# mhozza/covest

Hardware: AMD Instinct MI355X
Metric: grid-point log-likelihood evals/s, repeat model, 10k-bin hist (higher is better)
Workload: dtype f64

## Files before the change

### covest_amd/csrc/ll_factored.hip

```cpp
#include <hip/hip_runtime.h>

#include <algorithm>
#include <mutex>
#include <type_traits>

#include "direct_point.h"
#include "fastmath.h"
#include "kernels.h"
#include "point_fetch.h"
#include "streams.h"
#include "wave.h"

namespace covest {

namespace {

typedef double d4 __attribute__((ext_vector_type(4)));

constexpr double kShareScale = 0x1p128;


template <int N, int MU>
__device__ __forceinline__ void contract_step(int i, const double *cur, const int (&a_off)[MU], const int (&cut)[MU],
                                              const double (&r4)[MU], double (&wrun)[MU], d4 (&acc)[MU])
{
    double a[N];
#pragma unroll
    for (int k = 0; k < N; ++k)
        a[k] = cur[a_off[k] + 4 * i];
#pragma unroll
    for (int k = 0; k < N; ++k) {
        const double w = (i < cut[k]) ? wrun[k] : 0.0;
        wrun[k] *= r4[k];
        acc[k] = __builtin_amdgcn_mfma_f64_16x16x4f64(a[k], w, acc[k], 0, 0, 0);
    }
}

[[maybe_unused]] constexpr int kLdWide = 290;
template <int NT, int HU, bool TAIL, bool PLAIN, int LDC = 0>
__global__ __launch_bounds__(NT) void ll_factored_kernel(const DevModel m, const int32_t n_tiles, const int32_t n_items,
                                                         const double *__restrict__ tile_dbl,
                                                         const int32_t *__restrict__ tile_int,
                                                         const FactoredPlan plan,
                                                         double *__restrict__ out_ll, const SubList sub_list)
{
    const TileView tv = tile_view_from(n_tiles, n_items, tile_dbl, tile_int);
#ifdef COVEST_DIAG
    const long long dgx_0 = (long long)clock64();
    long long dgx_1 = 0, dgx_2 = 0, dgx_3 = 0, dgx_4 = 0;
#endif
    constexpr int NW = NT / kWave;
    constexpr int MU = 2 * HU;
    static_assert(MU == 6, "contract loops are written for 6 slots");
    constexpr bool SPO = PLAIN && TAIL;
    constexpr bool NEED_SCAL = !PLAIN;
    constexpr int LOG_DEG = PLAIN ? 3 : 5;
    const int LD = LDC ? LDC : plan.ld;
    constexpr int NE = FactoredLds::entries_of(NT);
    const FactoredLds lay{NT, plan.n_buf, LD, SPO};
    extern __shared__ double Gs[];
    __shared__ __attribute__((aligned(16))) double log_tab[kLogTableDoubles];
    __shared__ unsigned sub_rec[NE * 2];
    __shared__ __attribute__((aligned(16))) double2 rowc[2][kTileBins];
    __shared__ __attribute__((aligned(16))) double rows[NEED_SCAL ? 2 : 1][NEED_SCAL ? kTileBins : 2];
    __shared__ __attribute__((aligned(16))) double rho_tab[PLAIN ? NW * MU * 4 : 4];
    __shared__ double lconst_s;
    static_assert(MU == kMaxUnits, "the LDS layout counts kMaxUnits slots a wave");
    static_assert(sizeof(log_tab) + sizeof(sub_rec) + sizeof(rowc) + sizeof(rows) + sizeof(rho_tab) + sizeof(lconst_s) + 6 * 15 <=
                      kFactoredStaticLds, "the planners' LDS budget (tiles.h) must hold the kernel's static LDS");

    const int tid = threadIdx.x;
    const int lane = tid & (kWave - 1);
    const int wave = __builtin_amdgcn_readfirstlane(tid / kWave);
    const double p_clamp = plan.p_clamp;
    const double zero_frac = kZeroSteps * (kGridStep / p_clamp);
    const int list_mode = PLAIN ? 0 : plan.list_mode;

    const int n_seg = list_mode ? plan.n_seg : 1;
    const int unit = list_mode ? (int)blockIdx.x / n_seg : (int)blockIdx.x;
    const int seg = list_mode ? (int)blockIdx.x - unit * n_seg : 0;
    const int seg_items = (n_items + n_seg - 1) / n_seg;
    const int t_begin = seg * seg_items, t_end = min(n_items, t_begin + seg_items);
    const int64_t ce = (PLAIN || list_mode == 0) ? plan.ce_end - 1 - unit : plan.ce_begin + unit;
    const bool list = list_mode == 1 || list_mode == 2;
    const int64_t ic = list ? ce : ce / plan.n_e;
    const int64_t ie = list ? ce : ce - ic * plan.n_e;
    double par[kMaxParams] = {plan.c_axis[ic], plan.e_axis[ie], 0, 0, 0};
    constexpr int kLogPerThread = (kLogTableDoubles + NT - 1) / NT;
    double log_v[kLogPerThread];
#pragma unroll
    for (int u = 0; u < kLogPerThread; ++u)
        log_v[u] = kLogTable[min(tid + u * NT, kLogTableDoubles - 1)];
    const double rho_v = PLAIN ? plan.unit_rho[(int64_t)blockIdx.y * NW * MU * 4 + min(tid, NW * MU * 4 - 1)] : 0.0;
    double lc_first = 0.0;
    if (wave == NW - 1 && t_begin + lane < t_end)
        lc_first = tv.item_lconst[t_begin + lane];
#pragma unroll
    for (int u = 0; u < kLogPerThread; ++u)
        if (tid + u * NT < kLogTableDoubles)
            log_tab[tid + u * NT] = log_v[u];
    if (PLAIN && tid < NW * MU * 4)
        rho_tab[tid] = rho_v;
#pragma unroll
    for (int u = 0; u < (NE + NT - 1) / NT; ++u)
        if (tid + u * NT < NE) {
            sub_rec[2 * (tid + u * NT)] = 0xFFFFFFFFu;
            sub_rec[2 * (tid + u * NT) + 1] = 0;
        }
    clamp_point<2>(m, par);
    const bool finite = isfinite(par[0]) && isfinite(par[1]);
    const int n_pass = PLAIN ? 1 : plan.n_pass;
    if (tid < 8 * n_pass)
        Gs[lay.rates() + tid] = error_class_rate_mul(m, par[0], par[1], tid, m.n_err);
    if (wave == NW - 1) {
        double lc = 0.0 + lc_first;
        for (int t = t_begin + lane + kWave; t < t_end; t += kWave)
            lc += tv.item_lconst[t];
        lc = wave_sum(lc);
        if (lane == 0)
            lconst_s = PLAIN ? lc - kLogRawBias<kScaleBits> * tv.suf_h[0] : lc;
    }
    __syncthreads();
#ifdef COVEST_DIAG
    dgx_1 = (long long)clock64();
#endif

    const int my_pass = n_pass == 1 ? 0 : tid / plan.pass_stride;
    const int o_local = n_pass == 1 ? tid : tid - my_pass * plan.pass_stride;
    const bool wave_builds = wave * kWave < plan.n_columns;
    const int o_base = PLAIN ? 0 : list_mode == 2 ? plan.item_obase[ce] : plan.o_base;
    const int o_mine = o_base + o_local + 1;
    double lam[8];
#pragma unroll
    for (int s = 0; s < 8; ++s)
        lam[s] = Gs[lay.rates() + 8 * my_pass + s];
    double n_total = -1.0;
    if (n_pass > 1) {
        n_total = 0.0;
        for (int s = 0; s < 8 * n_pass; ++s)
            n_total += m.comb[s] * (1.0 - exp_neg_rn((double)o_mine * Gs[lay.rates() + s]));
    }
    __syncthreads();
    StreamSet<8> st;
    if (wave_builds) {
        st.template init<false>(m, lam, o_mine, finite && my_pass < n_pass && o_local < plan.max_o, log_tab,
                                log_tab, 8 * my_pass, n_total);
    } else {
        st.gone = 0u;
#pragma unroll
        for (int s = 0; s < 8; ++s) {
            st.v[s] = 0.0;
            st.x[s] = 0.0;
            st.an.set(s, 0.0, -INFINITY);
        }
    }
#ifdef COVEST_DIAG
    dgx_2 = (long long)clock64();
#endif
    const bool lane_in_row = tid < LD - 2;
    if (tid < FactoredLds::kSlack)
        Gs[lay.slack() + tid] = 0.0;
    if (tid < lay.rows()) {
        Gs[lay.pad(tid)] = 0.0;
        Gs[lay.pad(tid) + 1] = 0.0;
    }

    const int col = lane & 15;
    const int kq = lane >> 4;
    int len[MU], cont[MU], uhalf[MU], qslot[MU], cut[MU], a_off0[MU], nsh[MU];
    double r4[MU], llacc[MU];
    uint64_t dead[MU];
    unsigned off_slots = 0;
    bool newly_dead = false;
    CompSum spacc[(TAIL && !SPO) ? MU : 1];
    CompSum so = {0.0, 0.0};
    auto wave_block = [&](int w) -> int {
        if (list)
            return w >= NW - 2 ? 1 + 2 * (int)ce + (w - (NW - 2)) : 0;
        return (int)blockIdx.y * NW + w;
    };
    const int slot_base = wave_block(wave) * MU;
    int u_qt[MU], u_s0[MU], u_len[MU], u_cont[MU], u_half[MU], u_nsh[MU], u_o0[MU], u_T[MU];
#pragma unroll
    for (int k = 0; k < MU; ++k) {
        const int at = slot_base + k;
        u_qt[k] = plan.unit_tile[at];
        u_s0[k] = plan.unit_s0[at];
        u_len[k] = plan.unit_len[at];
        u_cont[k] = plan.unit_cont[at];
        u_half[k] = plan.unit_half[at];
        u_nsh[k] = PLAIN ? plan.unit_nsh[at] : 0;
        u_o0[k] = plan.unit_o0[at];
    }
#pragma unroll
    for (int k = 0; k < MU; ++k) {
        const int qt = __builtin_amdgcn_readfirstlane(u_qt[k]);
        const bool on = qt >= 0;
        const int slot = (on ? qt : 0) * 16 + col;
        qslot[k] = on ? slot : -1;
        u_T[k] = plan.q_T[slot];
        r4[k] = plan.q_r4[slot];
    }
#pragma unroll
    for (int k = 0; k < MU; ++k) {
        const bool on = qslot[k] >= 0;
        const int first_step = __builtin_amdgcn_readfirstlane(u_s0[k]);
        len[k] = __builtin_amdgcn_readfirstlane(u_len[k]);
        cont[k] = __builtin_amdgcn_readfirstlane(u_cont[k]);
        uhalf[k] = __builtin_amdgcn_readfirstlane(u_half[k]);
        nsh[k] = PLAIN ? __builtin_amdgcn_readfirstlane(u_nsh[k]) : 0;
        a_off0[k] = (16 * uhalf[k] + col) * LD + kq + 4 * first_step;
        const int t_lane = on ? u_T[k] : 0;
        const int o0 = __builtin_amdgcn_readfirstlane(u_o0[k]);
        cut[k] = ((t_lane - (o0 + kq) + 3) >> 2) - nsh[k];
        llacc[k] = 0.0;
        dead[k] = 0;
        spacc[(TAIL && !SPO) ? k : 0].hi = 0.0;
        spacc[(TAIL && !SPO) ? k : 0].lo = 0.0;
    }

    unsigned m_first = 0, m_cont = 0, m_sh = 0;
#pragma unroll
    for (int k = 0; k < MU; ++k) {
        m_first |= (qslot[k] >= 0 && !cont[k]) ? 1u << k : 0u;
        m_cont |= cont[k] ? 1u << k : 0u;
        m_sh |= nsh[k] > 0 ? 1u << k : 0u;
    }
    double wfirst[MU], wrun[MU];
    auto load_weights = [&]() {
#pragma unroll
        for (int k = 0; k < MU; ++k) {
            const double2 pw = reinterpret_cast<const double2 *>(plan.piece_w)[(int64_t)(slot_base + k) * kWave + lane];
            wfirst[k] = pw.x;
            wrun[k] = pw.y;
        }
    };
    load_weights();

    long long dg_a = 0, dg_b = 0, dg_b0 = 0, dg_c = 0, dg_w = 0, dg_t0 = 0, dg_zero = 0, dg_enter = 0, dg_first = 0;
#ifdef COVEST_DIAG
    const bool diag = plan.diag != nullptr;
#else
    constexpr bool diag = false;
#endif
    auto walk_tile = [&](auto n_tag, double *colp, double renorm, double k0) __attribute__((always_inline)) -> double {
        constexpr int N = decltype(n_tag)::value;
        if (!lane_in_row)
            return 0.0;
        double xx[8];
#pragma unroll
        for (int s = 0; s < 8; ++s) {
            double xs = st.x[s];
            if (s < N) {
                asm volatile("" : "+v"(xs));
                xx[s] = xs * xs;
            } else {
                xx[s] = 0.0;
            }
        }
        double *row = colp;
        double tsum = 0.0;
        if (SPO) {
            double kk = k0;
#pragma unroll
            for (int b = 0; b < kTileBins; b += 2) {
                double g1, g2;
                st.template step2n<N>(xx, g1, g2);
                row[0] = g1;
                row[LD] = g2;
                row += 2 * LD;
                tsum = fma(tsum, kk, g1);
                kk += 1.0;
                tsum = fma(tsum, kk, g2);
                kk += 1.0;
            }
            tsum *= renorm;
        } else {
#pragma unroll
            for (int b = 0; b < kTileBins; b += 2) {
                double g1, g2;
                st.template step2n<N>(xx, g1, g2);
                row[0] = g1;
                row[LD] = g2;
                row += 2 * LD;
            }
        }
        st.template leave_tile_n<N>(renorm);
        return tsum;
    };
    auto build_tile = [&](int t, bool seg_start, double *dst) __attribute__((always_inline)) -> double {
        if (COVEST_SKIP_PHASE(plan, 1))
            return 0.0;
        const TileRec rc = tv.rec[t];
        const double k0 = rc.k0;
        const int nb = rc.nb;
        const int n_live = st.enter_tile(k0 - 1.0, k0 + (double)(nb - 1), rc.lgam_prev, rc.lgam_last,
                                         rc.run_start != 0 || seg_start);
        if (diag) {
            const long long now__ = (long long)clock64();
            dg_enter += now__ - dg_t0;
            dg_t0 = now__;
        }
        double *colp = dst + (lane_in_row ? tid : 0);
        const double *scal = tv.scal + (int64_t)t * kTileBins;
        if (nb == kTileBins && !(SPO && rc.has_filler != 0)) {
            if (n_live > 4)
                return walk_tile(std::integral_constant<int, 8>{}, colp, rc.renorm, k0);
            if (n_live > 2)
                return walk_tile(std::integral_constant<int, 4>{}, colp, rc.renorm, k0);
            if (n_live == 2)
                return walk_tile(std::integral_constant<int, 2>{}, colp, rc.renorm, k0);
            if (n_live == 1)
                return walk_tile(std::integral_constant<int, 1>{}, colp, rc.renorm, k0);
            if (lane_in_row) {
                if (diag)
                    dg_zero += 1;
#pragma unroll
                for (int b = 0; b < kTileBins; ++b)
                    colp[b * LD] = 0.0;
            }
            return 0.0;
        }
        double tsum = 0.0;
        for (int b = 0; b < kTileBins; ++b) {
            const double g = b < nb ? st.step() : 0.0;
            if (SPO && b < nb)
                tsum = fma(g, scal[b], tsum);
            if (lane_in_row)
                colp[b * LD] = g;
        }
        st.leave_tile(rc.renorm);
        return tsum * 0x1p476;
    };
    auto sum_tile = [&](auto n_tag, const double *scal_ptr, double scal_or_k0, double renorm) __attribute__((always_inline)) -> double {
        constexpr int N = decltype(n_tag)::value;
        double xx[8];
#pragma unroll
        for (int s = 0; s < 8; ++s) {
            double xs = st.x[s];
            if (s < N) {
                asm volatile("" : "+v"(xs));
                xx[s] = xs * xs;
            } else {
                xx[s] = 0.0;
            }
        }
        double gsum = 0.0;
        if (SPO) {
            double kk = scal_or_k0;
#pragma unroll
            for (int b = 0; b < kTileBins; b += 2) {
                double g1, g2;
                st.template step2n<N>(xx, g1, g2);
                gsum = fma(gsum, kk, g1);
                kk += 1.0;
                gsum = fma(gsum, kk, g2);
                kk += 1.0;
            }
            st.template leave_tile_n<N>(renorm);
            return gsum * renorm;
        }
        const double *scal = SPO ? nullptr : scal_ptr;
#pragma unroll
        for (int half = 0; half < 2; ++half) {
            double sc[16];
#pragma unroll
            for (int b = 0; b < 16; ++b)
                sc[b] = scal[16 * half + b];
            asm volatile("" ::: "memory");
#pragma unroll
            for (int b = 0; b < 16; b += 2) {
                double g1, g2;
                st.template step2n<N>(xx, g1, g2);
                gsum = fma(g1, sc[b], gsum);
                gsum = fma(g2, sc[b + 1], gsum);
            }
        }
        st.template leave_tile_n<N>(renorm);
        return gsum * (1.0 / kBasicScale);
    };
    auto build_tile_sum = [&](int t, bool seg_start) __attribute__((always_inline)) -> double {
        const TileRec rc = tv.rec[t];
        const double k0 = rc.k0;
        const int nb = rc.nb;
        const int n_live = SPO ? st.enter_sum_tile(k0 - 1.0, k0 + (double)(nb - 1), rc.lgam_prev, rc.lgam_last,
                                                   rc.run_start != 0 || seg_start)
                               : st.enter_tile(k0 - 1.0, k0 + (double)(nb - 1), rc.lgam_prev, rc.lgam_last,
                                               rc.run_start != 0 || seg_start);
        const double *scal = tv.scal + (int64_t)t * kTileBins;
        if (nb == kTileBins && !(SPO && rc.has_filler != 0)) {
            if (n_live > 2)
                return sum_tile(std::integral_constant<int, 8>{}, scal, k0, rc.renorm);
            if (n_live == 2)
                return sum_tile(std::integral_constant<int, 2>{}, scal, k0, rc.renorm);
            if (n_live == 1)
                return sum_tile(std::integral_constant<int, 1>{}, scal, k0, rc.renorm);
            return 0.0;
        }
        double gsum = 0.0;
        for (int b = 0; b < nb; ++b)
            gsum = fma(st.step(), scal[b], gsum);
        st.leave_tile(rc.renorm);
        return SPO ? gsum * 0x1p476 : gsum * (1.0 / kBasicScale);
    };
    bool resync = false;
    auto build_item = [&](int it, bool seg_start, double *dst) __attribute__((always_inline)) {
        const int first = TAIL ? __builtin_amdgcn_readfirstlane(tv.item_first[it]) : it;
        if (TAIL && tv.item_sum[it] != 0) {
            if (COVEST_SKIP_PHASE(plan, 1))
                return;
            const int n = __builtin_amdgcn_readfirstlane(tv.item_ntiles[it]);
            if (SPO) {
                if (!seg_start) {
                    const int tl = first + n - 1;
                    const TileRec ra = tv.rec[first], rb = tv.rec[tl];
                    const double ka = ra.k0 - 1.0, kb = rb.k0 + (double)(rb.nb - 1);
                    const double lga = ra.lgam_prev, lgb = rb.lgam_last;
                    bool matters = false;
#pragma unroll
                    for (int s = 0; s < 8; ++s) {
                        if ((st.gone >> s) & 1u)
                            continue;
                        const double lx = st.an.lx(s), c = st.an.c(s);
                        const double top = fmax(fma(ka, lx, c - lga), fma(kb, lx, c - lgb));
                        matters = matters || !(top < StreamSet<8>::kSumWindowLn) || (st.x[s] >= ka - 1.0 && st.x[s] <= kb + 1.0);
                    }
                    if (!__any(matters)) {
#pragma unroll
                        for (int s = 0; s < 8; ++s)
                            st.v[s] = 0.0;
                        resync = true;
                        return;
                    }
                }
                for (int r = 0; r < n; ++r) {
                    if (st.gone == 0xFFu && !(seg_start && r == 0))
                        break;
                    so.add(build_tile_sum(first + r, (seg_start && r == 0) || resync));
                    resync = false;
                }
                return;
            }
            double *colp = dst + (lane_in_row ? tid : 0);
            for (int r = 0; r < n; ++r) {
                const double gsum = build_tile_sum(first + r, seg_start && r == 0);
                if (lane_in_row)
                    colp[r * LD] = gsum;
            }
            for (int r = n; r < kTileBins; ++r)
                if (lane_in_row)
// ... 473 lines not shown
    }
    ll = wave_sum(ll);
    double tail_term = 0.0;
    if (m.tail != 0.0) {
        double s = wave_comp_sum(sp);
        if (!(s < 1.0))
            s = 1.0;
        if (s < 1.0)
            tail_term = m.tail * log(1.0 - s);
    }
    if (__ballot(dead))
        ll = isnan(ll) ? ll : -INFINITY;
    double v = ll + tail_term;
    if (__ballot(poisoned) || !(isfinite(par[0]) && isfinite(par[1])))
        v = NAN;
    return v;
}

__global__ __launch_bounds__(kWave) void ll_finish_partials(const DevModel m, const int32_t n_tiles, const int32_t n_items,
                                                           const double *__restrict__ tile_dbl,
                                                           const int32_t *__restrict__ tile_int,
                                                           const double *__restrict__ partial,
                                                           const int32_t *__restrict__ first_item,
                                                           const double *__restrict__ point_par,
                                                           const int32_t *__restrict__ point_T, double *__restrict__ out_ll)
{
    const TileView tv = tile_view_from(n_tiles, n_items, tile_dbl, tile_int);
    const int p = blockIdx.x;
    const int c0 = first_item[p], c1 = first_item[p + 1];
    const int64_t n_rows = (int64_t)n_items * kTileBins;
    double par[kMaxParams];
#pragma unroll
    for (int d = 0; d < kMaxParams; ++d)
        par[d] = point_par[(int64_t)p * kMaxParams + d];
    clamp_point<5>(m, par);
    const double v = finish_point(m, tv, par, point_T[p], [&](int64_t row) {
        double pj = 0.0;
        for (int c = c0; c < c1; ++c)
            pj += partial[(int64_t)c * n_rows + row];
        return pj;
    });
    if (threadIdx.x == 0)
        out_ll[p] = v;
}

__global__ __launch_bounds__(kWave) void ll_finish_dense(const DevModel m, const int32_t n_tiles, const int32_t n_items,
                                                        const double *__restrict__ tile_dbl,
                                                        const int32_t *__restrict__ tile_int, const PointSource src,
                                                        const double *__restrict__ partial, const int64_t ce_first,
                                                        const int64_t n_cols, const int32_t *__restrict__ q_orig,
                                                        const int64_t n_q, const int64_t flat_end,
                                                        double *__restrict__ out_ll)
{
    const TileView tv = tile_view_from(n_tiles, n_items, tile_dbl, tile_int);
    const int64_t ce_local = blockIdx.x / n_cols, slot = blockIdx.x - ce_local * n_cols;
    const int32_t qo = q_orig[slot];
    if (qo < 0)
        return;
    const int64_t flat = (ce_first + ce_local) * n_q + qo;
    if (flat < src.flat_begin || flat >= flat_end)
        return;
    double par[kMaxParams];
    int T;
    fetch_point<5>(src, flat - src.flat_begin, par, T);
    clamp_point<5>(m, par);
    const int64_t n_rows = (int64_t)n_items * kTileBins;
    const double *mine = partial + (ce_local * n_cols + slot) * n_rows;
    const double v = finish_point(m, tv, par, T, [&](int64_t row) { return mine[row]; });
    if (threadIdx.x == 0)
        out_ll[flat - src.flat_begin] = v;
}

#endif

}

inline int64_t factored_rows_per_launch(const FactoredPlan &plan) { return std::max<int64_t>(1, ((int64_t)1 << 22) / plan.n_qblocks); }

template <int NT, bool TAIL, bool PLAIN, int LDC = 0>
hipError_t launch_ll_factored_variant(const DevModel &m, const TileView &tv, const FactoredPlan &plan,
                                      double *out_ll, const SubList &sub_list, hipStream_t stream)
{
    constexpr int HU = kHalfUnits;
    const FactoredLds lay{NT, plan.n_buf, plan.ld, PLAIN && TAIL};
    if (!lay.fits())
        return hipErrorInvalidValue;
    const size_t lds = (size_t)lay.total() * sizeof(double);
    static size_t configured[64] = {0};
    static std::mutex configured_lock;
    std::lock_guard<std::mutex> guard(configured_lock);
    int dev = 0;
    if (hipGetDevice(&dev) != hipSuccess || dev < 0 || dev >= 64)
        dev = 0;
    if (lds > configured[dev]) {
        hipError_t e = hipFuncSetAttribute(reinterpret_cast<const void *>(&ll_factored_kernel<NT, HU, TAIL, PLAIN, LDC>),
                                           hipFuncAttributeMaxDynamicSharedMemorySize, (int)lds);
        if (e != hipSuccess)
            return e;
        configured[dev] = lds;
    }
    const int64_t per_launch = factored_rows_per_launch(plan);
    for (int64_t first = plan.ce_begin; first < plan.ce_end; first += per_launch) {
        FactoredPlan part = plan;
        part.ce_begin = first;
        part.ce_end = std::min(plan.ce_end, first + per_launch);
        const dim3 grid((unsigned)((part.ce_end - part.ce_begin) * (plan.list_mode ? plan.n_seg : 1)),
                        (unsigned)plan.n_qblocks);
        hipLaunchKernelGGL((ll_factored_kernel<NT, HU, TAIL, PLAIN, LDC>), grid, dim3(NT), lds, stream, m, tv.n_tiles, tv.n_items,
                           tv.dbl_base, tv.int_base, part, out_ll, sub_list);
    }
    return hipGetLastError();
}

#ifdef COVEST_FACTORED_VARIANT
#if COVEST_FACTORED_VARIANT >= 8
template hipError_t launch_ll_factored_variant<512, (COVEST_FACTORED_VARIANT & 1) != 0, true, kLdWide>(
    const DevModel &, const TileView &, const FactoredPlan &, double *, const SubList &, hipStream_t);
#else
template hipError_t launch_ll_factored_variant<(COVEST_FACTORED_VARIANT & 4) ? 512 : 256, (COVEST_FACTORED_VARIANT & 2) != 0,
                                               (COVEST_FACTORED_VARIANT & 1) != 0>(const DevModel &, const TileView &,
                                                                                   const FactoredPlan &, double *,
                                                                                   const SubList &, hipStream_t);
#endif
#else
extern template hipError_t launch_ll_factored_variant<256, false, false>(const DevModel &, const TileView &, const FactoredPlan &, double *, const SubList &, hipStream_t);
extern template hipError_t launch_ll_factored_variant<256, false, true>(const DevModel &, const TileView &, const FactoredPlan &, double *, const SubList &, hipStream_t);
extern template hipError_t launch_ll_factored_variant<256, true, false>(const DevModel &, const TileView &, const FactoredPlan &, double *, const SubList &, hipStream_t);
extern template hipError_t launch_ll_factored_variant<256, true, true>(const DevModel &, const TileView &, const FactoredPlan &, double *, const SubList &, hipStream_t);
extern template hipError_t launch_ll_factored_variant<512, false, false>(const DevModel &, const TileView &, const FactoredPlan &, double *, const SubList &, hipStream_t);
extern template hipError_t launch_ll_factored_variant<512, false, true>(const DevModel &, const TileView &, const FactoredPlan &, double *, const SubList &, hipStream_t);
extern template hipError_t launch_ll_factored_variant<512, true, false>(const DevModel &, const TileView &, const FactoredPlan &, double *, const SubList &, hipStream_t);
extern template hipError_t launch_ll_factored_variant<512, true, true>(const DevModel &, const TileView &, const FactoredPlan &, double *, const SubList &, hipStream_t);
extern template hipError_t launch_ll_factored_variant<512, false, true, kLdWide>(const DevModel &, const TileView &, const FactoredPlan &, double *, const SubList &, hipStream_t);
extern template hipError_t launch_ll_factored_variant<512, true, true, kLdWide>(const DevModel &, const TileView &, const FactoredPlan &, double *, const SubList &, hipStream_t);
const char *const kFactoredVariantNames[kFactoredVariants] = {
    "ll_factored<256>", "ll_factored<256,plain>", "ll_factored<256,tail>", "ll_factored<256,tail,plain>",
    "ll_factored<512>", "ll_factored<512,plain>", "ll_factored<512,tail>", "ll_factored<512,tail,plain>",
    "ll_factored<512,plain,ld290>", "ll_factored<512,tail,plain,ld290>"};
const char *const kFactoredFinishNames[2] = {"ll_finish_dense", "ll_finish_partials"};
static_assert(kLdWide == 290, "kFactoredVariantNames spell the row stride of kLdWide");

namespace {

constexpr bool lds_overlap(int a0, int a1, int b0, int b1) { return a0 < b1 && b0 < a1; }
constexpr bool factored_lds_sound()
{
    for (int nt = 256; nt <= 512; nt += 256)
        for (int n_buf = 1; n_buf <= 2; ++n_buf)
            for (int k = 1; k <= 17; ++k)
                for (int spo = 0; spo <= 1; ++spo)
                    for (int t_end = 1; t_end <= 2; ++t_end) {
                        const FactoredLds l{nt, n_buf, kTileBins * k + 2, spo != 0};
                        const int ne = l.entries(), total = l.total();
                        if (l.buf(n_buf - 1) + kTileBins * l.ld > l.slack() || l.slack() + FactoredLds::kSlack > total ||
                            l.rates() + FactoredLds::kRates > total || l.pad(l.rows() - 1) + 2 > l.slack())
                            return false;
                        if (l.part_ll() + ne > total || l.part_hi(t_end) + ne > total || l.part_lo(t_end) + ne > total ||
                            lds_overlap(l.part_ll(), l.part_ll() + ne, l.part_hi(t_end), l.part_lo(t_end) + ne))
                            return false;
                        if (spo) {
                            const int s0 = l.spo_parts(t_end), s1 = s0 + 2 * ne, live = l.buf(t_end);
                            if (s1 > total || lds_overlap(s0, s1, l.slack(), l.slack() + FactoredLds::kSlack) ||
                                lds_overlap(s0, s1, live, live + (n_buf == 2 ? kTileBins : 2) * l.ld))
                                return false;
                            const int other = l.buf(t_end + 1);
                            if (n_buf == 2 && s0 < l.slack() && (s0 < other || s1 > other + kTileBins * l.ld))
                                return false;
                        }
                        if (factored_n_buf(l.ld) == n_buf && !l.fits())
                            return false;
                    }
    return true;
}
static_assert(factored_lds_sound(), "K-factored's LDS layout (tiles.h FactoredLds)");
static_assert(FactoredLds{512, 2, kLdWide, false}.total() == 2 * kTileBins * kLdWide + FactoredLds::kSlack, "C3's LDS");

template <int NT>
hipError_t launch_nt(const DevModel &m, const TileView &tv, const FactoredPlan &plan, double *out_ll,
                     const SubList &sub_list, hipStream_t stream)
{
    const bool plain = plan.list_mode == 0 && plan.n_pass == 1;
    {
        const bool tail = m.tail != 0.0;
        const int v = NT == 512 && plain && plan.ld == kLdWide ? 8 + (tail ? 1 : 0)
                                                                : (NT == 512 ? 4 : 0) + (tail ? 2 : 0) + (plain ? 1 : 0);
        const int64_t rows = plan.ce_end - plan.ce_begin, per_launch = factored_rows_per_launch(plan);
        record_launch(kFactoredVariantNames[v], (rows + per_launch - 1) / per_launch);
    }
    if (NT == 512 && plain && plan.ld == kLdWide)
        return m.tail != 0.0 ? launch_ll_factored_variant<512, true, true, kLdWide>(m, tv, plan, out_ll, sub_list, stream)
                             : launch_ll_factored_variant<512, false, true, kLdWide>(m, tv, plan, out_ll, sub_list, stream);
    if (m.tail != 0.0)
        return plain ? launch_ll_factored_variant<NT, true, true>(m, tv, plan, out_ll, sub_list, stream)
                     : launch_ll_factored_variant<NT, true, false>(m, tv, plan, out_ll, sub_list, stream);
    return plain ? launch_ll_factored_variant<NT, false, true>(m, tv, plan, out_ll, sub_list, stream)
                 : launch_ll_factored_variant<NT, false, false>(m, tv, plan, out_ll, sub_list, stream);
}

}

hipError_t launch_ll_finish_partials(const DevModel &m, const TileView &tv, const double *partial,
                                     const int32_t *first_item, const double *point_par, const int32_t *point_T,
                                     int64_t n_points, double *out_ll, hipStream_t stream)
{
    if (n_points <= 0)
        return hipSuccess;
    record_launch(kFactoredFinishNames[1]);
    hipLaunchKernelGGL(ll_finish_partials, dim3((unsigned)n_points), dim3(kWave), 0, stream, m, tv.n_tiles, tv.n_items, tv.dbl_base,
                       tv.int_base, partial, first_item, point_par, point_T, out_ll);
    return hipGetLastError();
}

hipError_t launch_ll_finish_dense(const DevModel &m, const TileView &tv, const PointSource &src, const double *partial,
                                  int64_t ce_first, int64_t n_ce, int64_t n_cols, const int32_t *q_orig, int64_t n_q,
                                  int64_t flat_end, double *out_ll, hipStream_t stream)
{
    const int64_t per_launch = std::max<int64_t>(1, ((int64_t)1 << 24) / n_cols);
    for (int64_t first = 0; first < n_ce; first += per_launch) {
        const int64_t cnt = std::min(per_launch, n_ce - first);
        record_launch(kFactoredFinishNames[0]);
        hipLaunchKernelGGL(ll_finish_dense, dim3((unsigned)(cnt * n_cols)), dim3(kWave), 0, stream, m, tv.n_tiles, tv.n_items,
                           tv.dbl_base, tv.int_base, src, partial + first * n_cols * (int64_t)tv.n_items * kTileBins,
                           ce_first + first, n_cols, q_orig, n_q, flat_end, out_ll);
    }
    return hipGetLastError();
}

hipError_t launch_ll_factored(const DevModel &m, const TileView &tv, const FactoredPlan &plan,
                              double *out_ll, const SubList &sub_list, hipStream_t stream)
{
    if (plan.ce_end <= plan.ce_begin)
        return hipSuccess;
    if (m.kind != 1 || plan.n_columns > plan.n_threads || 8 * plan.n_pass < m.n_err)
        return hipErrorInvalidValue;
    if (plan.n_threads == 256 && plan.half_units == 3)
        return launch_nt<256>(m, tv, plan, out_ll, sub_list, stream);
    if (plan.n_threads == 512 && plan.half_units == 3)
        return launch_nt<512>(m, tv, plan, out_ll, sub_list, stream);
    return hipErrorInvalidValue;
}
#endif

}
```

### covest_amd/csrc/streams.h

```cpp
#pragma once
#include <hip/hip_runtime.h>

#include "device_model.h"
#include "fastmath.h"
#include "point_fetch.h"
#include "tiles.h"

namespace covest {

template <int S>
struct RegAnchors {
    double lx_[S], c_[S];
    __device__ __forceinline__ void set(int s, double lx, double c) { lx_[s] = lx; c_[s] = c; }
    __device__ __forceinline__ double lx(int s) const { return lx_[s]; }
    __device__ __forceinline__ double c(int s) const { return c_[s]; }
};

template <int S>
struct LdsAnchors {
    double *mine;
    int stride;
    __device__ __forceinline__ void set(int s, double lx, double c)
    {
        mine[(2 * s) * stride] = lx;
        mine[(2 * s + 1) * stride] = c;
    }
    __device__ __forceinline__ double lx(int s) const { return mine[(2 * s) * stride]; }
    __device__ __forceinline__ double c(int s) const { return mine[(2 * s + 1) * stride]; }
};

template <int S, class Anchors = RegAnchors<S>>
struct StreamSet {
    double v[S];
    double x[S];
    Anchors an;
    unsigned gone;

    template <bool CANCEL = true>
    __device__ __forceinline__ void init(const DevModel &m, const double *lam, int o, bool live, const double *log_tab,
                                         const double *norm_tab = nullptr, int s0 = 0, double total = -1.0)
    {
        double n_os[S];
        double tot = 0.0;
        gone = 0u;
#pragma unroll
        for (int s = 0; s < S; ++s) {
            x[s] = (double)o * lam[s];
            n_os[s] = m.comb[s0 + s] * (1.0 - exp_neg_rn(x[s]));
            tot += n_os[s];
        }
        if (total >= 0.0)
            tot = total;
        if (tot == 0.0)
            tot = 1.0;
        const double ln_tot = CANCEL ? fast_log(tot, log_tab) : 0.0;
#pragma unroll
        for (int s = 0; s < S; ++s) {
            v[s] = 0.0;
            if (live && x[s] > 0.0 && n_os[s] > 0.0) {
                const double lx = fast_log(x[s], log_tab);
                double c;
                if (CANCEL ? x[s] < 0.015625 : true) {
                    const double a = n_os[s] / tot;
                    c = a > 0.0 ? fast_log(a, log_tab) - log_trunc_norm(x[s], lx, norm_tab) : -INFINITY;
                } else if (x[s] <= 200.0) {
                    c = (m.ln_comb[s0 + s] - ln_tot) - x[s];
                } else {
                    c = (m.ln_comb[s0 + s] - ln_tot) - log_trunc_norm(x[s], lx, norm_tab);
                }
                if (c == -INFINITY)
                    x[s] = 0.0;
                an.set(s, c == -INFINITY ? 0.0 : lx, c);
            } else {
                x[s] = 0.0;
                an.set(s, 0.0, -INFINITY);
            }
        }
    }

    __device__ __forceinline__ int enter_tile(double km1, double klast, double lgam_prev,
                                              double lgam_last, bool run_start)
    {
        return enter_tile_n<S>(km1, klast, lgam_prev, lgam_last, run_start);
    }

    static constexpr double kSumWindowLn = -60.0;
    __device__ __forceinline__ int enter_sum_tile(double km1, double klast, double lgam_prev, double lgam_last, bool run_start)
    {
        return enter_tile_n<S, true>(km1, klast, lgam_prev, lgam_last, run_start);
    }

    template <int N, bool SUM_ONLY = false>
    __device__ __forceinline__ int enter_tile_n(double km1, double klast, double lgam_prev,
                                                double lgam_last, bool run_start)
    {
        uint64_t m_window[N], m_need[N], m_real[SUM_ONLY ? N : 1];
        double a0s[N];
        uint64_t any_need = 0;
#pragma unroll
        for (int s = 0; s < N; ++s) {
            m_window[s] = m_need[s] = 0;
            a0s[s] = 0.0;
            if ((gone >> s) & 1u)
                continue;
            const double lx = an.lx(s), c = an.c(s);
            const double a0 = fma(km1, lx, c - lgam_prev);
            const double a1 = fma(klast, lx, c - lgam_last);
            const double top = fmax(a0, a1);
            m_window[s] = __ballot(top > (SUM_ONLY ? kSumWindowLn : kWindowLn));
            if (SUM_ONLY) {
                m_real[s] = __ballot(top > kWindowLn);
                v[s] = (!(top > kSumWindowLn) && km1 >= x[s]) ? 0.0 : v[s];
            }
            m_need[s] = run_start ? m_window[s] : (__ballot(v[s] == 0.0) & m_window[s]);
            if (run_start)
                v[s] = 0.0;
            a0s[s] = a0;
            any_need |= m_need[s];
        }
        if (any_need != 0) {
            const uint64_t me = 1ull << (threadIdx.x & 63);
#pragma unroll
            for (int s = 0; s < N; ++s) {
                if (m_need[s] == 0)
                    continue;
                const double anchored = exp_scaled(a0s[s], kScaleBits);
                v[s] = (m_need[s] & me) ? anchored : v[s];
            }
        }
        int n_live = 0;
#pragma unroll
        for (int s = 0; s < N; ++s) {
            if ((gone >> s) & 1u)
                continue;
            const uint64_t m_on = __ballot(v[s] != 0.0);
            const uint64_t m_stay = (SUM_ONLY ? m_real[s] : m_window[s]) | __ballot(!(km1 >= x[s]));
            if (m_on != 0)
                n_live = s + 1;
            else if (m_stay == 0)
                gone |= 1u << s;
        }
        return n_live;
    }

    __device__ __forceinline__ void retire_at_run_start(double km1, double klast, double lgam_prev, double lgam_last)
    {
#pragma unroll
        for (int s = 0; s < S; ++s) {
            if ((gone >> s) & 1u)
                continue;
            const double lx = an.lx(s), c = an.c(s);
            const double a0 = fma(km1, lx, c - lgam_prev);
            const double a1 = fma(klast, lx, c - lgam_last);
            const bool in_window = fmax(a0, a1) > kWindowLn;
            if (!__any(in_window || !(km1 >= x[s]))) {
                gone |= 1u << s;
                v[s] = 0.0;
            }
        }
    }

    __device__ __forceinline__ double step()
    {
        v[0] *= x[0];
        double g = v[0];
#pragma unroll
        for (int s = 1; s < S; ++s) {
            v[s] *= x[s];
            g += v[s];
        }
        return g;
    }

    __device__ __forceinline__ void step2(const double (&xx)[S], double &g1, double &g2)
    {
        g1 = v[0] * x[0];
#pragma unroll
        for (int s = 1; s < S; ++s)
            g1 = fma(v[s], x[s], g1);
        v[0] *= xx[0];
        g2 = v[0];
#pragma unroll
        for (int s = 1; s < S; ++s) {
            v[s] *= xx[s];
            g2 += v[s];
        }
    }

    template <int N>
    __device__ __forceinline__ void step2n(const double (&xx)[S], double &g1, double &g2)
    {
        static_assert(N >= 1 && N <= S, "live streams");
        g1 = v[0] * x[0];
#pragma unroll
        for (int s = 1; s < N; ++s)
            g1 = fma(v[s], x[s], g1);
        v[0] *= xx[0];
        g2 = v[0];
#pragma unroll
        for (int s = 1; s < N; ++s) {
            v[s] *= xx[s];
            g2 += v[s];
        }
    }

    template <int N>
    __device__ __forceinline__ double step_n()
    {
        v[0] *= x[0];
        double g = v[0];
#pragma unroll
        for (int s = 1; s < N; ++s) {
            v[s] *= x[s];
            g += v[s];
        }
        return g;
    }

    __device__ __forceinline__ bool only_first_left() const { return (gone | 1u) == (~0u >> (32 - S)); }

    template <int N>
    __device__ __forceinline__ void leave_tile_n(double renorm)
    {
#pragma unroll
        for (int s = 0; s < N; ++s)
            v[s] *= renorm;
    }

    __device__ __forceinline__ void squares(double (&xx)[S]) const
    {
#pragma unroll
        for (int s = 0; s < S; ++s)
            xx[s] = x[s] * x[s];
    }

    __device__ __forceinline__ void leave_tile(double renorm)
    {
#pragma unroll
        for (int s = 0; s < S; ++s)
            v[s] *= renorm;
    }
};

}
```

### covest_amd/csrc/tiles.h

```cpp
#pragma once
#include <hip/hip_runtime_api.h>
#include <stdint.h>

namespace covest {

constexpr int kTileBins = 32;
constexpr int kScaleBits = 540;
constexpr double kScaleLn = 540.0 * 0.693147180559945309417232121458;
constexpr double kWindowLn = -760.0;
constexpr int kBasicShift = 64;
constexpr double kBasicScale = 0x1p64;

struct alignas(64) TileRec {
    double k0, lgam_prev, lgam_last, renorm;
    int32_t nb, run_start, all_zero, has_filler;
    double pad[2];
};
static_assert(sizeof(TileRec) == 64, "one cache line");

struct TileView {
    int32_t n_tiles;
    int32_t n_items;
    const double *dbl_base;
    const int32_t *int_base;
    const double *first_key;
    const int32_t *n_bins;
    const int32_t *run_start;
    const int32_t *all_zero;
    const int32_t *has_filler;
    const double *lgam_prev;
    const double *lgam_last;
    const double *renorm;
    const double *scal;
    const double *cnt;
    const double *item_cnt;
    const double *item_scal;
    const double *item_iscal;
    const double *item_lconst;
    const double *suf_h;
    const double *suf_jh;
    const double *suf_lgh;
    const double *suf_first;
    const double *suf_first_lg;
    const double *last_key;
    const int32_t *item_first;
    const int32_t *item_ntiles;
    const int32_t *item_sum;
    const int32_t *row_bin;
    const TileRec *rec;
};

inline __host__ __device__ int64_t tile_arrays_dbl(int32_t nt, int32_t ni)
{
    const int64_t n = 4 * (int64_t)nt + 2 * (int64_t)nt * kTileBins + 3 * (int64_t)ni * kTileBins + ni + 5 * ((int64_t)nt + 1) + 2;
    return (n + 7) / 8 * 8;
}
inline __host__ __device__ int64_t tile_dbl_count(int32_t nt, int32_t ni) { return tile_arrays_dbl(nt, ni) + 8 * (int64_t)nt; }
inline __host__ __device__ int64_t tile_int_count(int32_t nt, int32_t ni) { return 4 * (int64_t)nt + 3 * (int64_t)ni + (int64_t)nt * kTileBins; }

inline __host__ __device__ TileView tile_view_from(int32_t nt, int32_t ni, const double *dbl, const int32_t *ints)
{
    TileView tv;
    tv.n_tiles = nt;
    tv.n_items = ni;
    tv.dbl_base = dbl;
    tv.int_base = ints;
    tv.first_key = dbl;
    tv.lgam_prev = dbl + nt;
    tv.lgam_last = dbl + 2 * (int64_t)nt;
    tv.renorm = dbl + 3 * (int64_t)nt;
    tv.scal = dbl + 4 * (int64_t)nt;
    tv.cnt = tv.scal + (int64_t)nt * kTileBins;
    tv.item_cnt = tv.cnt + (int64_t)nt * kTileBins;
    tv.item_scal = tv.item_cnt + (int64_t)ni * kTileBins;
    tv.item_iscal = tv.item_scal + (int64_t)ni * kTileBins;
    tv.item_lconst = tv.item_iscal + (int64_t)ni * kTileBins;
    tv.suf_h = tv.item_lconst + ni;
    tv.suf_jh = tv.suf_h + (nt + 1);
    tv.suf_lgh = tv.suf_jh + (nt + 1);
    tv.suf_first = tv.suf_lgh + (nt + 1);
    tv.suf_first_lg = tv.suf_first + (nt + 1);
    tv.last_key = tv.suf_first_lg + (nt + 1);
    tv.n_bins = ints;
    tv.run_start = ints + nt;
    tv.all_zero = ints + 2 * (int64_t)nt;
    tv.has_filler = ints + 3 * (int64_t)nt;
    tv.item_first = ints + 4 * (int64_t)nt;
    tv.item_ntiles = tv.item_first + ni;
    tv.item_sum = tv.item_ntiles + ni;
    tv.row_bin = tv.item_sum + ni;
    tv.rec = reinterpret_cast<const TileRec *>(dbl + tile_arrays_dbl(nt, ni));
    return tv;
}

constexpr int kMaxUnits = 6;
constexpr int kHalfUnits = 3;
constexpr int kBuildCost = 18;
constexpr int kBuildCostLowKeys = 24;
constexpr int kLowKeyTile = 384;
#ifndef COVEST_LIST_SEGMENTS
#define COVEST_LIST_SEGMENTS 16
#endif
constexpr int kListSegments = COVEST_LIST_SEGMENTS;
constexpr int kMinPieceSteps = 6;
constexpr int kSharedStepsPerMfma = 4;
constexpr int kMinSharedSteps = 3;
constexpr int kLastBuilderExtra = 4;
constexpr int kUnitOverhead = 2;

struct FactoredPlan {
    const double *c_axis, *e_axis;
    int64_t n_e;
    int64_t ce_begin, ce_end;
    int64_t n_q;
    int32_t n_qtiles;
    int32_t max_o;
    int32_t n_pass;
    int32_t pass_stride;
    int32_t n_columns;
    int32_t o_base;
    int32_t n_threads;
    int32_t half_units;
    int32_t n_qblocks;
    int32_t ld;
    int32_t n_buf;
    const int32_t *unit_tile;
    const int32_t *unit_half;
    const int32_t *unit_s0;
    const int32_t *unit_o0;
    const int32_t *unit_len;
    const int32_t *unit_cont;
    const int32_t *unit_nsh;
    const int32_t *unit_pair;
    const double *unit_rho;
    const double *piece_w;
    const int32_t *qtile_nsteps;
    const int32_t *qtile_nfull;
    const int32_t *q_T;
    const int32_t *q_orig;
    const double *q_first8;
    const double *q_r4;
    int64_t flat_begin, flat_end;
    int32_t list_mode;
    double p_clamp;
    int32_t n_seg;
    const int32_t *item_obase;
    double *partial;
    int64_t ce_first;
    int64_t n_cols_partial;
    long long *diag;
    int32_t skip_phases;
};

constexpr int kLdsBytes = 160 * 1024;
constexpr int kFactoredStaticLds = 13440;

constexpr __host__ __device__ int factored_ld(int columns) { return (columns + kTileBins - 1) / kTileBins * kTileBins + 2; }

struct FactoredLds {
    int nt, n_buf, ld;
    bool spo;
    static constexpr int kSlack = 64;
    static constexpr int kRates = 32;
    __host__ __device__ static constexpr int entries_of(int nt) { return nt / 64 * kMaxUnits * 16; }
    __host__ __device__ constexpr int entries() const { return entries_of(nt); }
    __host__ __device__ constexpr int rows() const { return n_buf * kTileBins; }
    __host__ __device__ constexpr int buf(int b) const { return n_buf == 2 ? (b & 1) * kTileBins * ld : 0; }
    __host__ __device__ constexpr int pad(int row) const { return row * ld + ld - 2; }
    __host__ __device__ constexpr int slack() const { return n_buf * kTileBins * ld; }
    __host__ __device__ constexpr int rates() const { return 0; }
    __host__ __device__ constexpr bool spo_inside() const
    {
        return kTileBins * ld >= (n_buf == 2 ? 0 : 2 * ld) + 3 * entries();
    }
    __host__ __device__ constexpr int spo_parts(int t_end) const
    {
        return !spo_inside() ? slack() + kSlack : n_buf == 2 ? buf(t_end + 1) + entries() : 2 * ld + entries();
    }
    __host__ __device__ constexpr int part_ll() const { return 0; }
    __host__ __device__ constexpr int part_hi(int t_end) const { return spo ? spo_parts(t_end) : entries(); }
    __host__ __device__ constexpr int part_lo(int t_end) const { return part_hi(t_end) + entries(); }
    __host__ __device__ constexpr int total() const
    {
        const int a = slack() + kSlack, b = 3 * entries(), c = spo && !spo_inside() ? slack() + kSlack + 2 * entries() : 0;
        return a > b ? (a > c ? a : c) : (b > c ? b : c);
    }
    __host__ __device__ constexpr bool fits() const { return total() * (int)sizeof(double) + kFactoredStaticLds <= kLdsBytes; }
};

constexpr __host__ __device__ int factored_n_buf(int ld) { return FactoredLds{512, 2, ld, true}.fits() ? 2 : 1; }

#ifdef COVEST_DIAG
#define COVEST_SKIP_PHASE(plan, bits) (((plan).skip_phases & (bits)) != 0)
#else
#define COVEST_SKIP_PHASE(plan, bits) false
#endif

}
```

Measured before the change: 398.1 million.

## Add per-tile relative window table to skip negligible streams in plain kernel

Adds a pre-pass in the plain factored kernel where each building wave scans tiles and records, per tile, the largest log-term margin over the window from reference lanes, using an LDS table updated with atomicMax. When entering a tile, streams whose top term falls below that reference minus a fixed margin (about 100 bits) are excluded from the window, so fewer streams are live and fewer walk_tile steps run. The cost is an extra per-block pass over tiles with atomics and a barrier, plus 128 more LDS doubles. There is a risk of dropping terms if the margin argument does not hold.

```diff
diff --git a/covest_amd/csrc/ll_factored.hip b/covest_amd/csrc/ll_factored.hip
--- a/covest_amd/csrc/ll_factored.hip
+++ b/covest_amd/csrc/ll_factored.hip
@@ -37,6 +37,7 @@
 }
 
 [[maybe_unused]] constexpr int kLdWide = 290;
+[[maybe_unused]] constexpr double kWindowMargin = 100.0 * 0.693147180559945309417232121458 + 2.07944154167983592825169636437;
 template <int NT, int HU, bool TAIL, bool PLAIN, int LDC = 0>
 __global__ __launch_bounds__(NT) void ll_factored_kernel(const DevModel m, const int32_t n_tiles, const int32_t n_items,
                                                          const double *__restrict__ tile_dbl,
@@ -101,6 +102,8 @@
             log_tab[tid + u * NT] = log_v[u];
     if (PLAIN && tid < NW * MU * 4)
         rho_tab[tid] = rho_v;
+    if (PLAIN && tid < FactoredLds::kWinTiles)
+        Gs[lay.win() + tid] = 0.0;
 #pragma unroll
     for (int u = 0; u < (NE + NT - 1) / NT; ++u)
         if (tid + u * NT < NE) {
@@ -153,6 +156,34 @@
             st.x[s] = 0.0;
             st.an.set(s, 0.0, -INFINITY);
         }
+    }
+    if (PLAIN) {
+        if (wave_builds) {
+            unsigned long long *wtab = reinterpret_cast<unsigned long long *>(Gs + lay.win());
+            const double lx0 = st.an.lx(0), c0 = st.an.c(0), x0 = st.x[0], lam0 = lam[0];
+            const bool ref_lane = o_mine >= 3 && x0 > 0.0;
+            const bool lowest = o_mine == 3, highest = o_mine == plan.max_o;
+            for (int base = t_begin; base < t_end; base += kWave) {
+                const int it_l = min(base + lane, t_end - 1);
+                const int t_l = TAIL ? tv.item_first[it_l] : it_l;
+                const bool use_l = base + lane < t_end && !(TAIL && tv.item_sum[it_l] != 0) && t_l < FactoredLds::kWinTiles;
+                const double km1_l = tv.first_key[t_l] - 1.0, klast_l = km1_l + (double)tv.n_bins[t_l];
+                const double lgp_l = tv.lgam_prev[t_l], lgl_l = tv.lgam_last[t_l];
+                const uint64_t use = __ballot(use_l);
+                const int n = min(kWave, t_end - base);
+                for (int j = 0; j < n; ++j) {
+                    if (!((use >> j) & 1))
+                        continue;
+                    const double km1 = wave_bcast(km1_l, j), klast = wave_bcast(klast_l, j);
+                    const int t = __builtin_amdgcn_readlane(t_l, j);
+                    const double r = fmin(fma(km1, lx0, c0 - wave_bcast(lgp_l, j)), fma(klast, lx0, c0 - wave_bcast(lgl_l, j))) - kWindowLn;
+                    const bool cand = (x0 >= km1 - lam0 && x0 <= klast + lam0) || (lowest && x0 > klast) || (highest && x0 < km1);
+                    if (ref_lane && cand && r > 0.0)
+                        atomicMax(&wtab[t], ((unsigned long long)__double_as_longlong(r) & ~1023ull) | (unsigned long long)o_mine);
+                }
+            }
+        }
+        __syncthreads();
     }
 #ifdef COVEST_DIAG
     dgx_2 = (long long)clock64();
@@ -294,8 +325,21 @@
         const TileRec rc = tv.rec[t];
         const double k0 = rc.k0;
         const int nb = rc.nb;
-        const int n_live = st.enter_tile(k0 - 1.0, k0 + (double)(nb - 1), rc.lgam_prev, rc.lgam_last,
-                                         rc.run_start != 0 || seg_start);
+        int n_live;
+        if constexpr (PLAIN) {
+            double thr = kWindowLn;
+            if (t < FactoredLds::kWinTiles) {
+                const unsigned long long ref =
+                    reinterpret_cast<const unsigned long long *>(Gs + FactoredLds{NT, plan.n_buf, LD, SPO}.win())[t];
+                const double over = __longlong_as_double((long long)(ref & ~1023ull)) - kWindowMargin;
+                thr = (tid >= (int)(ref & 1023ull) && over > 0.0) ? kWindowLn + over : kWindowLn;
+            }
+            n_live = st.enter_tile(k0 - 1.0, k0 + (double)(nb - 1), rc.lgam_prev, rc.lgam_last,
+                                   rc.run_start != 0 || seg_start, RelWindow{thr});
+        } else {
+            n_live = st.enter_tile(k0 - 1.0, k0 + (double)(nb - 1), rc.lgam_prev, rc.lgam_last,
+                                   rc.run_start != 0 || seg_start);
+        }
         if (diag) {
             const long long now__ = (long long)clock64();
             dg_enter += now__ - dg_t0;
@@ -1075,7 +1119,8 @@
                     for (int t_end = 1; t_end <= 2; ++t_end) {
                         const FactoredLds l{nt, n_buf, kTileBins * k + 2, spo != 0};
                         const int ne = l.entries(), total = l.total();
-                        if (l.buf(n_buf - 1) + kTileBins * l.ld > l.slack() || l.slack() + FactoredLds::kSlack > total ||
+                        if (l.buf(n_buf - 1) + kTileBins * l.ld > l.slack() || l.slack() + FactoredLds::kSlack > l.win() ||
+                            l.win() + FactoredLds::kWinTiles > total ||
                             l.rates() + FactoredLds::kRates > total || l.pad(l.rows() - 1) + 2 > l.slack())
                             return false;
                         if (l.part_ll() + ne > total || l.part_hi(t_end) + ne > total || l.part_lo(t_end) + ne > total ||
@@ -1083,7 +1128,7 @@
                             return false;
                         if (spo) {
                             const int s0 = l.spo_parts(t_end), s1 = s0 + 2 * ne, live = l.buf(t_end);
-                            if (s1 > total || lds_overlap(s0, s1, l.slack(), l.slack() + FactoredLds::kSlack) ||
+                            if (s1 > total || lds_overlap(s0, s1, l.slack(), l.win() + FactoredLds::kWinTiles) ||
                                 lds_overlap(s0, s1, live, live + (n_buf == 2 ? kTileBins : 2) * l.ld))
                                 return false;
                             const int other = l.buf(t_end + 1);
@@ -1096,7 +1141,9 @@
     return true;
 }
 static_assert(factored_lds_sound(), "K-factored's LDS layout (tiles.h FactoredLds)");
-static_assert(FactoredLds{512, 2, kLdWide, false}.total() == 2 * kTileBins * kLdWide + FactoredLds::kSlack, "C3's LDS");
+static_assert(FactoredLds{512, 2, kLdWide, false}.total() ==
+                  2 * kTileBins * kLdWide + FactoredLds::kSlack + FactoredLds::kWinTiles, "C3's LDS");
+static_assert(FactoredLds{512, 2, kLdWide, true}.fits(), "the widest double-buffered shape holds the window table too");
 
 template <int NT>
 hipError_t launch_nt(const DevModel &m, const TileView &tv, const FactoredPlan &plan, double *out_ll,
diff --git a/covest_amd/csrc/streams.h b/covest_amd/csrc/streams.h
--- a/covest_amd/csrc/streams.h
+++ b/covest_amd/csrc/streams.h
@@ -27,6 +27,14 @@
     }
     __device__ __forceinline__ double lx(int s) const { return mine[(2 * s) * stride]; }
     __device__ __forceinline__ double c(int s) const { return mine[(2 * s + 1) * stride]; }
+};
+
+struct AbsWindow {
+    static constexpr bool kRelative = false;
+};
+struct RelWindow {
+    static constexpr bool kRelative = true;
+    double thr;
 };
 
 template <int S, class Anchors = RegAnchors<S>>
@@ -78,10 +86,11 @@
         }
     }
 
+    template <class Win = AbsWindow>
     __device__ __forceinline__ int enter_tile(double km1, double klast, double lgam_prev,
-                                              double lgam_last, bool run_start)
-    {
-        return enter_tile_n<S>(km1, klast, lgam_prev, lgam_last, run_start);
+                                              double lgam_last, bool run_start, Win win = Win())
+    {
+        return enter_tile_n<S, false, Win>(km1, klast, lgam_prev, lgam_last, run_start, win);
     }
 
     static constexpr double kSumWindowLn = -60.0;
@@ -90,10 +99,11 @@
         return enter_tile_n<S, true>(km1, klast, lgam_prev, lgam_last, run_start);
     }
 
-    template <int N, bool SUM_ONLY = false>
+    template <int N, bool SUM_ONLY = false, class Win = AbsWindow>
     __device__ __forceinline__ int enter_tile_n(double km1, double klast, double lgam_prev,
-                                                double lgam_last, bool run_start)
-    {
+                                                double lgam_last, bool run_start, Win win = Win())
+    {
+        static_assert(!(SUM_ONLY && Win::kRelative), "a sum tile's window is absolute");
         uint64_t m_window[N], m_need[N], m_real[SUM_ONLY ? N : 1];
         double a0s[N];
         uint64_t any_need = 0;
@@ -108,11 +118,14 @@
             const double a1 = fma(klast, lx, c - lgam_last);
             const double top = fmax(a0, a1);
             m_window[s] = __ballot(top > (SUM_ONLY ? kSumWindowLn : kWindowLn));
+            uint64_t m_enter = m_window[s];
+            if constexpr (Win::kRelative)
+                m_enter &= __ballot(top > win.thr || klast >= x[s]);
             if (SUM_ONLY) {
                 m_real[s] = __ballot(top > kWindowLn);
                 v[s] = (!(top > kSumWindowLn) && km1 >= x[s]) ? 0.0 : v[s];
             }
-            m_need[s] = run_start ? m_window[s] : (__ballot(v[s] == 0.0) & m_window[s]);
+            m_need[s] = run_start ? m_enter : (__ballot(v[s] == 0.0) & m_enter);
             if (run_start)
                 v[s] = 0.0;
             a0s[s] = a0;
diff --git a/covest_amd/csrc/tiles.h b/covest_amd/csrc/tiles.h
--- a/covest_amd/csrc/tiles.h
+++ b/covest_amd/csrc/tiles.h
@@ -162,12 +162,15 @@
     bool spo;
     static constexpr int kSlack = 64;
     static constexpr int kRates = 32;
+    static constexpr int kWinTiles = 128;
     __host__ __device__ static constexpr int entries_of(int nt) { return nt / 64 * kMaxUnits * 16; }
     __host__ __device__ constexpr int entries() const { return entries_of(nt); }
     __host__ __device__ constexpr int rows() const { return n_buf * kTileBins; }
     __host__ __device__ constexpr int buf(int b) const { return n_buf == 2 ? (b & 1) * kTileBins * ld : 0; }
     __host__ __device__ constexpr int pad(int row) const { return row * ld + ld - 2; }
     __host__ __device__ constexpr int slack() const { return n_buf * kTileBins * ld; }
+    __host__ __device__ constexpr int win() const { return slack() + kSlack; }
+    __host__ __device__ constexpr int tail_end() const { return win() + kWinTiles; }
     __host__ __device__ constexpr int rates() const { return 0; }
     __host__ __device__ constexpr bool spo_inside() const
     {
@@ -175,14 +178,14 @@
     }
     __host__ __device__ constexpr int spo_parts(int t_end) const
     {
-        return !spo_inside() ? slack() + kSlack : n_buf == 2 ? buf(t_end + 1) + entries() : 2 * ld + entries();
+        return !spo_inside() ? tail_end() : n_buf == 2 ? buf(t_end + 1) + entries() : 2 * ld + entries();
     }
     __host__ __device__ constexpr int part_ll() const { return 0; }
     __host__ __device__ constexpr int part_hi(int t_end) const { return spo ? spo_parts(t_end) : entries(); }
     __host__ __device__ constexpr int part_lo(int t_end) const { return part_hi(t_end) + entries(); }
     __host__ __device__ constexpr int total() const
     {
-        const int a = slack() + kSlack, b = 3 * entries(), c = spo && !spo_inside() ? slack() + kSlack + 2 * entries() : 0;
+        const int a = tail_end(), b = 3 * entries(), c = spo && !spo_inside() ? tail_end() + 2 * entries() : 0;
         return a > b ? (a > c ? a : c) : (b > c ? b : c);
     }
     __host__ __device__ constexpr bool fits() const { return total() * (int)sizeof(double) + kFactoredStaticLds <= kLdsBytes; }
```

Result: slower. 367.8 million (-7.6%).
